# danilodjor/fault-tolerant-llm-training

Measured on AMD Instinct MI355X. Metric: tokens/sec/GPU seq-len 2048 DP at 1/2/4/8 MI355X; checkpoint save wall-clock (s), higher is better.
Workload: dtype bf16; 1 GPU; model=llama3-8b, global_batch=1, seq_len=2048, parallelism=dp1

## Files before the change

csrc/kernels/embedding.hip:

```cpp
#include "torch_utils.h"

#include <algorithm>

namespace {

__global__ __launch_bounds__(256) void emb_fwd_kernel(const int64_t* __restrict__ tok,
                                                      const char* __restrict__ w,
                                                      char* __restrict__ out, int T, int row_bytes) {
  const int row = blockIdx.x;
  const int64_t t = tok[row];
  const uint4* src = reinterpret_cast<const uint4*>(w + t * (long)row_bytes);
  uint4* dst = reinterpret_cast<uint4*>(out + (long)row * row_bytes);
  for (int c = threadIdx.x; c < row_bytes / 16; c += blockDim.x) dst[c] = src[c];
}

constexpr int SORT_NT = 1024, SORT_W = SORT_NT / 64, SORT_BITS = 6, SORT_BINS = 1 << SORT_BITS;

__global__ __launch_bounds__(SORT_NT) void tok_sort_kernel(const int64_t* __restrict__ tok, int T, int passes,
                                                           int* __restrict__ keys, int* __restrict__ vals) {
  __shared__ int hist[SORT_BINS];
  __shared__ int start[SORT_BINS];
  __shared__ int rbase[SORT_BINS];
  __shared__ int wcnt[SORT_W][SORT_BINS];
  const int tid = threadIdx.x, lane = tid & 63, wid = tid >> 6;
// ... 26 lines not shown
      const int d = (k >> shift) & (SORT_BINS - 1);
      unsigned long long m = __ballot(valid);
#pragma unroll
      for (int b = 0; b < SORT_BITS; ++b) {
        const unsigned long long bb = __ballot(valid && ((d >> b) & 1));
        m &= ((d >> b) & 1) ? bb : ~bb;
      }
      const int rank = __popcll(m & lower);
      wcnt[wid][lane] = 0;
      __syncthreads();
      if (valid && rank == 0) wcnt[wid][d] = __popcll(m);
      __syncthreads();
      if (tid < SORT_BINS) {
        int s = 0;
        for (int w = 0; w < SORT_W; ++w) {
          const int c = wcnt[w][tid];
          wcnt[w][tid] = s;
          s += c;
        }
        rbase[tid] = start[tid];
        start[tid] += s;
      }
      __syncthreads();
      if (valid) {
        const int pos = rbase[d] + wcnt[wid][d] + rank;
        dk[pos] = k;
        dv[pos] = v;
      }
      __syncthreads();
    }
  }
}

template <class E>
__global__ __launch_bounds__(256) void emb_bwd_kernel(const int* __restrict__ sorted_tok,
                                                      const int* __restrict__ perm,
                                                      const typename E::T* __restrict__ dy,
                                                      typename E::T* __restrict__ dw, int T, int D,
                                                      bool accumulate) {
  const int wave = (blockIdx.x * blockDim.x + threadIdx.x) >> 6;
  const int lane = threadIdx.x & 63;
  if (wave >= T) return;
  const int t = sorted_tok[wave];
  if (wave > 0 && sorted_tok[wave - 1] == t) return;
  int end = wave + 1;
  while (end < T && sorted_tok[end] == t) ++end;
  typename E::T* dst = dw + t * (long)D;
  for (int c = lane * 8; c < D; c += 64 * 8) {
    float acc[8] = {0, 0, 0, 0, 0, 0, 0, 0};
    for (int k = wave; k < end; ++k) {
      float x[8];
      ld8<E>(dy + perm[k] * (long)D + c, x);
#pragma unroll
      for (int j = 0; j < 8; ++j) acc[j] += x[j];
    }
    if (accumulate) {
      float o[8];
      ld8<E>(dst + c, o);
#pragma unroll
      for (int j = 0; j < 8; ++j) acc[j] += o[j];
    }
    st8<E>(dst + c, acc);
  }
}

template <class E>
__global__ __launch_bounds__(256) void emb_bwd_sq_kernel(const int* __restrict__ sorted_tok,
                                                         const int* __restrict__ perm,
                                                         const typename E::T* __restrict__ dy,
                                                         typename E::T* __restrict__ dw, int T, int D,
                                                         float* __restrict__ part, int nparts) {
  __shared__ float red[4];
  const int lane = threadIdx.x & 63, wid = threadIdx.x >> 6;
  float sq = 0.f;
  for (int wave = blockIdx.x * 4 + wid; wave < T; wave += gridDim.x * 4) {
    const int t = sorted_tok[wave];
    if (wave > 0 && sorted_tok[wave - 1] == t) continue;
    int end = wave + 1;
    while (end < T && sorted_tok[end] == t) ++end;
    typename E::T* dst = dw + t * (long)D;
    for (int c = lane * 8; c < D; c += 64 * 8) {
      float acc[8] = {0, 0, 0, 0, 0, 0, 0, 0};
      for (int k = wave; k < end; ++k) {
        float x[8];
        ld8<E>(dy + perm[k] * (long)D + c, x);
#pragma unroll
        for (int j = 0; j < 8; ++j) acc[j] += x[j];
      }
      const P8<E> r = pk8<E>(acc);
      *reinterpret_cast<uint4*>(dst + c) = r.v[0];
      if constexpr (!E::is16) *reinterpret_cast<uint4*>(dst + c + 4) = r.v[1];
      float st[8];
      unp8<E>(r, st);
#pragma unroll
      for (int j = 0; j < 8; ++j) sq = fmaf(st[j], st[j], sq);
    }
  }
  const float tot = block_sum<256>(sq, red);
  if (threadIdx.x == 0) part[blockIdx.x] = tot;
  for (long i = blockIdx.x + (long)gridDim.x * (1 + threadIdx.x); i < nparts; i += (long)gridDim.x * 256)
    part[i] = 0.f;
}

}

at::Tensor embedding_fwd(const at::Tensor& tokens, const at::Tensor& weight) {
  FT_CHECK_CUDA(weight);
  FT_CHECK_MODEL_DTYPE(weight);
  FT_CHECK_CONTIG(weight);
  FT_CHECK_CONTIG(tokens);
  TORCH_CHECK(tokens.scalar_type() == at::kLong, "embedding: tokens must be int64");
  const int D = weight.size(1);
  TORCH_CHECK(D % 8 == 0, "embedding: dim must be a multiple of 8");
  const int T = tokens.numel();
  const at::DeviceGuard guard(weight.device());
  auto sizes = tokens.sizes().vec();
  sizes.push_back(D);
  auto out = at::empty(sizes, weight.options());
  if (T > 0)
    hipLaunchKernelGGL(emb_fwd_kernel, dim3(T), dim3(256), 0, ft_stream(), cptr<int64_t>(tokens),
                       cptr<char>(weight), mptr<char>(out), T, (int)(D * weight.element_size()));
  FT_LAUNCH_CHECK();
  return out;
}

void embedding_bwd_(const at::Tensor& dy, const at::Tensor& tokens, const at::Tensor& dw,
                    bool accumulate, const std::optional<at::Tensor>& part) {
  FT_CHECK_CUDA(dy);
  FT_CHECK_MODEL_DTYPE(dy);
  TORCH_CHECK(dy.scalar_type() == dw.scalar_type(), "embedding_bwd: dtype mismatch");
  FT_CHECK_CONTIG(dy);
  FT_CHECK_CONTIG(dw);
  const int D = dw.size(1);
  const int T = tokens.numel();
  TORCH_CHECK(dy.numel() == (long)T * D, "embedding_bwd: shape mismatch");
  const at::DeviceGuard guard(dw.device());
  TORCH_CHECK(tokens.scalar_type() == at::kLong, "embedding_bwd: tokens must be int64");
  const long V = dw.size(0);
  TORCH_CHECK(V >= 1 && V < (1L << 30), "embedding_bwd: vocabulary size out of range");
  int bits = 1;
  while ((1L << bits) < V) ++bits;
  const int passes = (bits + SORT_BITS - 1) / SORT_BITS;
  auto flat = tokens.reshape({-1}).contiguous();
  if (!accumulate) FT_HIP_CHECK(hipMemsetAsync(dw.data_ptr(), 0, dw.nbytes(), ft_stream()));
  if (T > 0) {
    auto kv = at::empty({4, (long)T}, tokens.options().dtype(at::kInt));
    int* keys = mptr<int>(kv);
    int* vals = keys + 2L * T;
    hipLaunchKernelGGL(tok_sort_kernel, dim3(1), dim3(SORT_NT), 0, ft_stream(), cptr<int64_t>(flat), T, passes,
                       keys, vals);
    FT_LAUNCH_CHECK();
    const long fin = (long)((passes - 1) & 1) * T;
    const int blocks = (T * 64 + 255) / 256;
    const bool sq = part.has_value() && part->defined();
    if (sq) {
      TORCH_CHECK(!accumulate, "embedding_bwd: norm partials need a fresh gradient");
      FT_CHECK_F32((*part));
      FT_CHECK_CONTIG((*part));
      const int np = (int)part->numel();
      const int g = std::max(1, std::min({blocks, 256, np}));
      FT_DISPATCH_E(dy.scalar_type(),
                    hipLaunchKernelGGL(emb_bwd_sq_kernel<E>, dim3(g), dim3(256), 0, ft_stream(), keys + fin,
                                       vals + fin, cptr<typename E::T>(dy), mptr<typename E::T>(dw), T, D,
                                       mptr<float>(*part), np));
    } else {
      FT_DISPATCH_E(dy.scalar_type(),
                    hipLaunchKernelGGL(emb_bwd_kernel<E>, dim3(blocks), dim3(256), 0, ft_stream(), keys + fin,
                                       vals + fin, cptr<typename E::T>(dy), mptr<typename E::T>(dw), T, D,
                                       accumulate));
    }
  } else if (part.has_value() && part->defined()) {
    part->zero_();
  }
  FT_LAUNCH_CHECK();
}

TORCH_LIBRARY_FRAGMENT(ftamd, m) {
  m.def("embedding_fwd(Tensor tokens, Tensor weight) -> Tensor", &embedding_fwd);
  m.def("embedding_bwd_(Tensor dy, Tensor tokens, Tensor(a!) dw, bool accumulate, Tensor(b!)? part=None) -> ()",
        &embedding_bwd_);
}
```

csrc/kernels/optim.hip:

```cpp
#include "torch_utils.h"

#include <vector>

#include <cstdlib>

namespace {

typedef unsigned int u32x4_t __attribute__((ext_vector_type(4)));

template <bool NT>
__device__ __forceinline__ uint4 ld16(const void* p) {
  if constexpr (NT) {
    const u32x4_t v = __builtin_nontemporal_load(reinterpret_cast<const u32x4_t*>(p));
    return make_uint4(v.x, v.y, v.z, v.w);
  } else {
    return *reinterpret_cast<const uint4*>(p);
  }
}

template <bool NT>
__device__ __forceinline__ void st16(void* p, uint4 v) {
  if constexpr (NT) {
    const u32x4_t w = {v.x, v.y, v.z, v.w};
    __builtin_nontemporal_store(w, reinterpret_cast<u32x4_t*>(p));
// ... 33 lines not shown
  }
  __shared__ float red[4];
  s = block_sum<256>(s, red);
  if (threadIdx.x == 0) partial[blockIdx.x] = s;
}

__global__ __launch_bounds__(1024) void norm_finish_kernel(const float* __restrict__ partial,
                                                           int np, float extra_sumsq_scale,
                                                           float max_norm,
                                                           float* __restrict__ stats) {
  float s = 0.f;
  const int n4 = np >> 2;
  const float4* p4 = reinterpret_cast<const float4*>(partial);
  if ((reinterpret_cast<uintptr_t>(partial) & 15) == 0) {
    for (int i = threadIdx.x; i < n4; i += 1024) {
      const float4 v = p4[i];
      s += (v.x + v.y) + (v.z + v.w);
    }
    for (int i = 4 * n4 + threadIdx.x; i < np; i += 1024) s += partial[i];
  } else {
    for (int i = threadIdx.x; i < np; i += 1024) s += partial[i];
  }
  __shared__ float red[16];
  s = block_sum<1024>(s, red);
  if (threadIdx.x == 0) {
    const float norm = sqrtf(s * extra_sumsq_scale);
    stats[0] = norm;
    const bool bad = !isfinite(norm);
    stats[1] = (max_norm > 0.f && !bad) ? fminf(1.f, max_norm / (norm + 1e-6f)) : 1.f;
    stats[2] = (bad || stats[2] != 0.f) ? 1.f : 0.f;
  }
}

template <class P, class S, bool NT>
__global__ __launch_bounds__(256) void adamw_kernel(typename P::T* __restrict__ p,
                                                    const typename P::T* __restrict__ g,
                                                    typename S::T* __restrict__ m,
                                                    typename S::T* __restrict__ v,
                                                    long n8, float lr, float beta1, float beta2,
                                                    float eps, float wd, float inv_bc1,
                                                    float inv_sqrt_bc2,
                                                    const float* __restrict__ stats,
                                                    const float* __restrict__ hyper, int exact) {
  if (stats[2] != 0.f) return;
  if (hyper != nullptr) {
    lr = hyper[0];
    inv_bc1 = hyper[1];
    inv_sqrt_bc2 = hyper[2];
  }
  const float coef = stats[1];
  const float decay = 1.f - lr * wd;
  const float step = lr * inv_bc1;
  for (long i = blockIdx.x * 256L + threadIdx.x; i < n8; i += (long)gridDim.x * 256) {
    float pf[8], gf[8], mf[8], vf[8];
    V8<P, NT>::load(p + i * 8, pf);
    V8<P, NT>::load(g + i * 8, gf);
    V8<S, NT>::load(m + i * 8, mf);
    V8<S, NT>::load(v + i * 8, vf);
#pragma unroll
    for (int j = 0; j < 8; ++j) {
      const float gj = gf[j] * coef;
      pf[j] *= decay;
      mf[j] += (gj - mf[j]) * (1.f - beta1);
      vf[j] = vf[j] * beta2 + (1.f - beta2) * gj * gj;
      if (exact) {
        const float denom = sqrtf(vf[j]) * inv_sqrt_bc2 + eps;
        pf[j] -= step * mf[j] / denom;
      } else {
        const float denom = fast_sqrt(vf[j]) * inv_sqrt_bc2 + eps;
        pf[j] -= step * mf[j] * fast_rcp(denom);
      }
    }
    V8<P, NT>::store(p + i * 8, pf);
    V8<S, NT>::store(m + i * 8, mf);
    V8<S, NT>::store(v + i * 8, vf);
  }
}

int stream_grid(long n8) {
  long g = (n8 + 255) / 256;
  return (int)std::max(1L, std::min(g, 65535L));
}

void launch_sumsq(const at::Tensor& grad, long n8, int nb, float* partial) {
  const bool nt = stream_nt();
  FT_DISPATCH_E(grad.scalar_type(), {
    if (nt)
      hipLaunchKernelGGL((sumsq_kernel<E, true>), dim3(nb), dim3(256), 0, ft_stream(),
                         cptr<typename E::T>(grad), n8, partial);
    else
      hipLaunchKernelGGL((sumsq_kernel<E, false>), dim3(nb), dim3(256), 0, ft_stream(),
                         cptr<typename E::T>(grad), n8, partial);
  });
}

}

void grad_norm_(const at::Tensor& grad, const at::Tensor& stats, double max_norm) {
  FT_CHECK_CUDA(grad);
  FT_CHECK_CONTIG(grad);
  FT_CHECK_F32(stats);
  TORCH_CHECK(grad.numel() % 8 == 0, "grad_norm: numel must be a multiple of 8");
  const at::DeviceGuard guard(grad.device());
  const long n8 = grad.numel() / 8;
  const int nb = std::max(1, std::min(NORM_BLOCKS, (int)((n8 + 255) / 256)));
  auto partial = at::empty({nb}, grad.options().dtype(at::kFloat));
  launch_sumsq(grad, n8, nb, mptr<float>(partial));
  FT_LAUNCH_CHECK();
  hipLaunchKernelGGL(norm_finish_kernel, dim3(1), dim3(1024), 0, ft_stream(), cptr<float>(partial), nb,
                     1.f, (float)max_norm, mptr<float>(stats));
  FT_LAUNCH_CHECK();
}

void adamw_(const at::Tensor& p, const at::Tensor& g, const at::Tensor& m, const at::Tensor& v,
            const at::Tensor& stats, double lr, double beta1, double beta2, double eps, double wd,
            int64_t step, int64_t max_blocks, const std::optional<at::Tensor>& hyper) {
  const float* hp = nullptr;
  if (hyper.has_value() && hyper->defined()) {
    FT_CHECK_F32((*hyper));
    TORCH_CHECK(hyper->is_cuda() && hyper->numel() >= 3, "adamw: hyper must be a device fp32[3]");
    hp = cptr<float>(*hyper);
  }
  FT_CHECK_CUDA(p);
  FT_CHECK_CONTIG(p);
  FT_CHECK_CONTIG(g);
  FT_CHECK_CONTIG(m);
  FT_CHECK_CONTIG(v);
  FT_CHECK_F32(stats);
  TORCH_CHECK(p.numel() == g.numel() && p.numel() == m.numel() && p.numel() == v.numel(),
              "adamw: size mismatch");
  TORCH_CHECK(p.numel() % 8 == 0, "adamw: numel must be a multiple of 8");
  TORCH_CHECK(p.scalar_type() == g.scalar_type() && m.scalar_type() == v.scalar_type(),
              "adamw: dtype mismatch");
  const at::DeviceGuard guard(p.device());
  const long n8 = p.numel() / 8;
  const float bc1 = 1.f - (float)std::pow(beta1, (double)step);
  const float bc2 = 1.f - (float)std::pow(beta2, (double)step);
  const float inv_bc1 = 1.f / bc1, inv_sqrt_bc2 = 1.f / std::sqrt(bc2);
  int nb = stream_grid(n8);
  if (max_blocks > 0) nb = (int)std::max(1L, std::min((n8 + 255) / 256, (long)max_blocks));
  const dim3 grid(nb), block(256);
  const bool nt = stream_nt();
  TORCH_CHECK(m.scalar_type() == p.scalar_type() || m.scalar_type() == at::kFloat,
              "adamw: optimizer states must have the parameter dtype or fp32");
  const int exact = (int)ft_exact_math() || p.scalar_type() == at::kFloat;
  auto go = [&](auto ptag, auto stag) {
    using P = decltype(ptag);
    using S = decltype(stag);
    using PT = typename P::T;
    using ST = typename S::T;
    if (nt)
      hipLaunchKernelGGL((adamw_kernel<P, S, true>), grid, block, 0, ft_stream(), mptr<PT>(p),
                         cptr<PT>(g), mptr<ST>(m), mptr<ST>(v), n8, (float)lr, (float)beta1,
                         (float)beta2, (float)eps, (float)wd, inv_bc1, inv_sqrt_bc2,
                         cptr<float>(stats), hp, exact);
    else
      hipLaunchKernelGGL((adamw_kernel<P, S, false>), grid, block, 0, ft_stream(), mptr<PT>(p),
                         cptr<PT>(g), mptr<ST>(m), mptr<ST>(v), n8, (float)lr, (float)beta1,
                         (float)beta2, (float)eps, (float)wd, inv_bc1, inv_sqrt_bc2,
                         cptr<float>(stats), hp, exact);
  };
  FT_DISPATCH_E(p.scalar_type(), {
    if (m.scalar_type() == at::kFloat) go(E{}, EF32{});
    else go(E{}, E{});
  });
  FT_LAUNCH_CHECK();
}

void sumsq_into_(const at::Tensor& grad, const at::Tensor& partial) {
  FT_CHECK_CUDA(grad);
  FT_CHECK_CONTIG(grad);
  FT_CHECK_F32(partial);
  FT_CHECK_CONTIG(partial);
  TORCH_CHECK(grad.numel() % 8 == 0, "sumsq_into: numel must be a multiple of 8");
  TORCH_CHECK(partial.numel() >= 1 && partial.numel() <= 65535, "sumsq_into: bad partial size");
  const at::DeviceGuard guard(grad.device());
  const long n8 = grad.numel() / 8;
  const int nb = (int)partial.numel();
  launch_sumsq(grad, n8, nb, mptr<float>(partial));
  FT_LAUNCH_CHECK();
}

void norm_finish_(const at::Tensor& partial, const at::Tensor& stats, double max_norm) {
  FT_CHECK_CUDA(partial);
  FT_CHECK_F32(partial);
  FT_CHECK_F32(stats);
  const at::DeviceGuard guard(partial.device());
  hipLaunchKernelGGL(norm_finish_kernel, dim3(1), dim3(1024), 0, ft_stream(), cptr<float>(partial),
                     (int)partial.numel(), 1.f, (float)max_norm, mptr<float>(stats));
  FT_LAUNCH_CHECK();
}

int64_t cu_masked_stream(int64_t stride, int64_t phase) {
  TORCH_CHECK(stride >= 1 && phase >= 0 && phase < stride, "cu_masked_stream: 0 <= phase < stride");
  int dev = 0, ncu = 0;
  FT_HIP_CHECK(hipGetDevice(&dev));
  FT_HIP_CHECK(hipDeviceGetAttribute(&ncu, hipDeviceAttributeMultiprocessorCount, dev));
  std::vector<uint32_t> mask((ncu + 31) / 32, 0u);
  for (int c = (int)phase; c < ncu; c += (int)stride) mask[c / 32] |= 1u << (c % 32);
  hipStream_t st = nullptr;
  FT_HIP_CHECK(hipExtStreamCreateWithCUMask(&st, (uint32_t)mask.size(), mask.data()));
  return reinterpret_cast<int64_t>(st);
}

TORCH_LIBRARY_FRAGMENT(ftamd, m) {
  m.def("cu_masked_stream(int stride, int phase=0) -> int", &cu_masked_stream);
  m.def("sumsq_into_(Tensor grad, Tensor(a!) partial) -> ()", &sumsq_into_);
  m.def("norm_finish_(Tensor partial, Tensor(a!) stats, float max_norm) -> ()", &norm_finish_);
  m.def("grad_norm_(Tensor grad, Tensor(a!) stats, float max_norm) -> ()", &grad_norm_);
  m.def(
      "adamw_(Tensor(a!) p, Tensor g, Tensor(b!) m, Tensor(c!) v, Tensor stats, float lr, float "
      "beta1, float beta2, float eps, float wd, int step, int max_blocks=0, Tensor? hyper=None) -> ()",
      &adamw_);
}
```

fault_tolerant_llm_training_amd/ckpt/state.py:

```python
from __future__ import annotations

import hashlib
from collections import OrderedDict
from dataclasses import asdict
from typing import Any, Dict, Optional

import torch

from .format import FORMAT_TAG, strip_compile_prefix


def layout_hash(model) -> str:
    flat = model.flat
    h = hashlib.sha1()
    for name, s in flat.slots.items():
        h.update(f"{name}:{s.shape}:{s.offset};".encode())
    h.update(str(flat.dtype).encode())
    return h.hexdigest()[:16]


def _view(buf: torch.Tensor, s) -> torch.Tensor:
    return buf[s.offset : s.offset + s.numel].view(s.shape)


# ... 25 lines not shown
    }
    if rng is not None:
        out["rng"] = rng
    return out


def _flat_source(tensors, slots, numel: int, dtype) -> Optional[torch.Tensor]:
    base = None
    for name, t in tensors.items():
        s = slots.get(name)
        if s is None or t.dtype != dtype or tuple(t.shape) != tuple(s.shape) or not t.is_contiguous():
            return None
        st = t.untyped_storage()
        if base is None:
            base = st
        elif st.data_ptr() != base.data_ptr():
            return None
        if t.storage_offset() != s.offset:
            return None
    if base is None or base.nbytes() < numel * torch.tensor([], dtype=dtype).element_size():
        return None
    return torch.empty(0, dtype=dtype).set_(base)[:numel]


@torch.no_grad()
def restore_model(model, sd: Dict[str, torch.Tensor]) -> str:
    flat = model.flat
    sd = strip_compile_prefix(sd)
    expected = list(model.state_dict().keys())
    missing = [k for k in expected if k not in sd]
    unexpected = [k for k in sd if k not in flat.slots]
    if missing or unexpected:
        raise KeyError(f"checkpoint/model mismatch: missing={missing[:5]} unexpected={unexpected[:5]}")
    src = _flat_source(sd, flat.slots, flat.numel, flat.dtype)
    if src is not None:
        from .restore import h2d

        h2d(flat.params, src)
        return "flat"
    for name in expected:
        _view(flat.params, flat.slots[name]).copy_(sd[name], non_blocking=True)
    return "per-tensor"


def capture_rng(device: torch.device) -> Dict[str, Any]:
    r = {"torch": torch.get_rng_state()}
    if device.type == "cuda":
        r["cuda"] = torch.cuda.get_rng_state(device)
    return r


def restore_rng(r: Optional[Dict[str, Any]], device: torch.device) -> None:
    if not r:
        return
    if "torch" in r:
        torch.set_rng_state(r["torch"])
    if device.type == "cuda" and "cuda" in r:
        torch.cuda.set_rng_state(r["cuda"], device)


def shard_regions(model, optimizer, rank: int, world: int, align: int = 2048):
    from .engine import Region

    flat = model.flat
    P = flat.numel

# ... 15 lines not shown
```

fault_tolerant_llm_training_amd/ops/functional.py:

```python
from __future__ import annotations

import collections
import functools
import os
from typing import Optional

import torch
import torch.nn.functional as F

from .._native import kernels, native
from .grad_sink import GradSink

IGNORE_INDEX = -100

_BLAS_ONLY = os.environ.get("FT_GEMM_BLAS", "0") == "1"
_W4_FWD = True
_W4_BWD = os.environ.get("FT_W4_BWD", "1") != "0"
_W4_DTYPES = (torch.bfloat16, torch.float16)
_F32_MFMA = os.environ.get("FT_F32_MFMA", "1") != "0"


def set_f32_mfma(on: bool) -> None:
    global _F32_MFMA
    _F32_MFMA = bool(on)
# ... 210 lines not shown

def join_dw_stream() -> None:
    if _dw_streams:
        cur = torch.cuda.current_stream()
        k = _dev_key(cur.device)
        s = _dw_streams.get(k)
        if s is not None:
            cur.wait_stream(s)
            q = _dw_pending.get(k)
            if q:
                q.clear()


def norm_bwd_into_sink(dy, x, w, rstd, mean, sink: GradSink, dres=None) -> torch.Tensor:
    dx = kernels().norm_bwd(dy, x, w, rstd, mean, sink.buf, dres, sink.accumulate, sink.part)
    if sink.part is not None:
        sink.sq_done = True
    sink.ready()
    return dx


def _write_weight_grad(sink: Optional[GradSink], g: torch.Tensor):
    if sink is None:
        return g
    sink.set_(g.to(sink.buf.dtype))
    return None


class EmbeddingFn(torch.autograd.Function):
    @staticmethod
    def forward(ctx, tokens, weight, sink):
        ctx.sink = sink
        ctx.vocab = weight.shape[0]
        ctx.save_for_backward(tokens)
        ctx.wshape = weight.shape
        if native(weight):
            return kernels().embedding_fwd(tokens.contiguous(), weight)
        return F.embedding(tokens, weight)

    @staticmethod
    def backward(ctx, dy):
        (tokens,) = ctx.saved_tensors
        sink = ctx.sink
        dy = dy.contiguous()
        if sink is not None and sink.gather is not None:
            if sink.defer:
                sink.stash.append((tokens.reshape(-1), dy.reshape(-1, dy.shape[-1])))
                return None, None, None
            if sink.stash:
                tokens = torch.cat([t for t, _ in sink.stash] + [tokens.reshape(-1)])
                dy = torch.cat([g for _, g in sink.stash] + [dy.reshape(-1, dy.shape[-1])])
                sink.stash = []
            tokens, dy = sink.gather(tokens, dy)
        if native(dy):
            if sink is None:
                dw = torch.zeros(ctx.wshape, dtype=dy.dtype, device=dy.device)
                kernels().embedding_bwd_(dy, tokens.contiguous(), dw, False)
                return None, dw, None
            part = sink.part if (sink.part is not None and not sink.accumulate) else None
            kernels().embedding_bwd_(dy, tokens.contiguous(), sink.buf, sink.accumulate, part)
            if part is not None:
                sink.sq_done = True
            sink.ready()
            return None, None, None
        dw = torch.zeros(ctx.wshape, dtype=torch.float32, device=dy.device)
        if dy.is_cuda:
            dw.index_put_((tokens.reshape(-1),), dy.reshape(-1, ctx.wshape[1]).float(), accumulate=True)
        else:
            dw.index_add_(0, tokens.reshape(-1), dy.reshape(-1, ctx.wshape[1]).float())
        return None, _write_weight_grad(sink, dw.to(dy.dtype)), None


def embedding(tokens, weight, sink=None):
    return EmbeddingFn.apply(tokens, weight, sink)


def norm_reference(x: torch.Tensor, w: torch.Tensor, eps: float, layernorm: bool) -> torch.Tensor:
    xf = x.float()
    if layernorm:
        xf = xf - xf.mean(-1, keepdim=True)
    n = xf * torch.rsqrt(xf.pow(2).mean(-1, keepdim=True) + eps)
    return n.type_as(x) * w


class NormFn(torch.autograd.Function):
    @staticmethod
    def forward(ctx, x, weight, sink, eps, layernorm):
        ctx.sink, ctx.eps, ctx.ln = sink, eps, layernorm
        if native(x):
            xc = x.contiguous()
            y, rstd, mean = kernels().norm_fwd(xc, weight, eps, layernorm)
            ctx.save_for_backward(xc, weight, rstd, mean)
            return y
# ... 360 lines not shown
```

fault_tolerant_llm_training_amd/ops/grad_sink.py:

```python
from __future__ import annotations

from typing import Callable, Optional

import torch


class GradSink:
    __slots__ = ("buf", "start", "end", "accumulate", "hook", "name", "gather", "defer", "stash", "part", "sq_done")

    def __init__(self, buf: torch.Tensor, start: int = 0, end: int = 0, name: str = ""):
        self.buf = buf
        self.start = start
        self.end = end
        self.accumulate = False
        self.hook: Optional[Callable[["GradSink"], None]] = None
        self.name = name
        self.gather: Optional[Callable] = None
        self.defer = False
        self.stash: list = []
        self.part: Optional[torch.Tensor] = None
        self.sq_done = False

    def ready(self) -> None:
        if self.hook is not None:
            self.hook(self)

    def mm(self, a: torch.Tensor, b: torch.Tensor) -> None:
        out = self.buf.view(a.shape[0], b.shape[1])
        if self.accumulate:
            out.addmm_(a, b)
        else:
            torch.mm(a, b, out=out)
        self.ready()

    def set_(self, g: torch.Tensor) -> None:
        if self.accumulate:
            self.buf.add_(g.view_as(self.buf))
        else:
            self.buf.copy_(g.view_as(self.buf))
        self.ready()


def sink_of(p: torch.Tensor) -> Optional[GradSink]:
    return getattr(p, "_ft_sink", None)
```

fault_tolerant_llm_training_amd/optim/adamw.py:

```python
from __future__ import annotations

import math
from typing import List, Optional, Tuple

import torch
import torch.distributed as dist

from .._native import kernels, native
from ..models.flat import FlatParamSpace


class NonFiniteGradError(RuntimeError):
    pass


class ParamGate:

    def __init__(self):
        self.entries: List[list] = []

    def add(self, lo: int, hi: int, handle) -> None:
        self.entries.append([lo, hi, handle])

    def wait(self, lo: int, hi: int) -> None:
# ... 55 lines not shown
        name_of = {id(p): n for n, p in flat.param_objs.items()}
        self._index_slots = [flat.slots[name_of[id(p)]] for p in params]

    def clip_grad_norm_(self, max_norm: Optional[float] = None) -> torch.Tensor:
        if max_norm is not None:
            self.max_grad_norm = float(max_norm)
        return self.stats[0]

    def _stream_ctx(self):
        r = self.reducer
        if r is not None and r.overlap:
            return torch.cuda.stream(r.side)
        import contextlib

        return contextlib.nullcontext()

    def _hyper(self):
        grp = self.param_groups[0]
        b1, b2 = grp["betas"]
        return float(grp["lr"]), b1, b2, grp["eps"], grp["weight_decay"]

    def stage_hyper(self, step: int) -> None:
        import numpy as np

        lr, b1, b2, _eps, _wd = self._hyper()
        bc1 = np.float32(1.0) - np.float32(b1 ** step)
        bc2 = np.float32(1.0) - np.float32(b2 ** step)
        h = self._hyper_ring[self._hyper_i % len(self._hyper_ring)]
        self._hyper_i += 1
        h.copy_(torch.from_numpy(np.array([np.float32(lr), np.float32(1.0) / bc1,
                                           np.float32(1.0) / np.sqrt(bc2)], dtype=np.float32)))
        self.hyper.copy_(h, non_blocking=True)

    def _update(self, p, g, m, v, lr, b1, b2, eps, wd, max_blocks: int = 0):
        if native(p):
            kernels().adamw_(p, g, m, v, self.stats, lr, b1, b2, eps, wd, self.step_count, max_blocks,
                             self.hyper if self.graph_mode else None)
        else:
            _adamw_reference(p, g, m, v, self.stats, lr, b1, b2, eps, wd, self.step_count)

    @torch.no_grad()
    def step(self, closure=None):
        self.step_count += 1
        lr, b1, b2, eps, wd = self._hyper()
        f = self.flat
        r = self.reducer
        cuda = f.params.is_cuda
        if r is None:
            if cuda:
                from ..ops.functional import join_dw_stream

                join_dw_stream()
            if native(f.grads):
                kernels().grad_norm_(f.grads, self.stats, self.max_grad_norm)
            else:
                gd = f.grads.double() if f.grads.dtype == torch.float64 else f.grads.float()
                _norm_reference(gd.pow(2).sum().reshape(1), self.stats, self.max_grad_norm)
            self._update(f.params, f.grads, self.exp_avg, self.exp_avg_sq, lr, b1, b2, eps, wd)
            self._publish_stats()
            return None
        if r.overlap:
            r.side.wait_stream(torch.cuda.current_stream())
        with self._stream_ctx():
            total = r.global_sumsq()
            if cuda:
                kernels().norm_finish_(total, self.stats, self.max_grad_norm)
            else:
                _norm_reference(total.sum().reshape(1), self.stats, self.max_grad_norm)
            if not self.graph_mode:
                self._publish_stats()
            for b in sorted(r.buckets, key=lambda b: b.lo):
                slo, shi = r.state_range(b)
                self._update(r.param_for_update(b), r.grad_for_update(b), self.exp_avg[slo:shi],
                             self.exp_avg_sq[slo:shi], lr, b1, b2, eps, wd,
                             self.overlap_blocks if r.overlap else 0)
                if self.zero1 and r.dry_comm:
                    pass
                elif self.zero1 and r.single_stream and r.overlap:
                    dist.all_gather_into_tensor(f.params[b.lo : b.hi], r.param_shard(b), group=r.group)
                    b.agevent.record()
                    self.gate.add(b.lo, b.hi, b.agevent)
                elif self.zero1:
                    work = dist.all_gather_into_tensor(f.params[b.lo : b.hi], r.param_shard(b),
                                                       group=r.group, async_op=True)
                    if r.overlap:
                        self.gate.add(b.lo, b.hi, work)
                    else:
                        work.wait()
                elif r.overlap:
                    b.event.record()
                    self.gate.add(b.lo, b.hi, b.event)
        return None

    def _publish_stats(self):
        i = self.step_count % self.RING
        h = self._ring[i]
        if self.stats.is_cuda:
            h.copy_(self.stats, non_blocking=True)
            ev = self._ring_events[i]
            if ev is None:
                ev = self._ring_events[i] = torch.cuda.Event()
            ev.record()
            self._stats_event = ev
        else:
            h.copy_(self.stats)
        self._ring_steps[i] = self.step_count
        self._stats_step = self.step_count

# ... 165 lines not shown
```

fault_tolerant_llm_training_amd/parallel/ddp.py:

```python
from __future__ import annotations

import os
from typing import List, Optional

import torch
import torch.distributed as dist

from .._native import kernels, native
from ..models.flat import FlatParamSpace
from ..ops.grad_sink import GradSink

MODES = ("local", "allreduce", "zero1")
LOCAL_BUCKET_MB = 64.0
DP_BUCKET_MB = 256.0
PARTIALS_PER_BUCKET = 512
SUMSQ_AT_END = False


def set_sumsq_at_end(on: bool) -> None:
    global SUMSQ_AT_END
    SUMSQ_AT_END = bool(on)


FUSED_SUMSQ = True


def set_fused_sumsq(on: bool) -> None:
    global FUSED_SUMSQ
    FUSED_SUMSQ = bool(on)


def sink_partials(numel: int, ndim: int, shape=None, tile_rows: int = 256) -> int:
    if ndim <= 1:
        return max(1, (numel + 31) // 32)
    n = max(1, (numel + 32767) // 32768)
    if shape is not None and len(shape) == 2:
        n = max(n, -(-int(shape[0]) // tile_rows) * -(-int(shape[1]) // 128))
    return n


def _copy_back(dst: torch.Tensor, src: torch.Tensor, temps) -> None:
    dst.copy_(src)
    if src.is_cuda:
        cur = torch.cuda.current_stream(src.device)
        for t in temps:
            t.record_stream(cur)


# ... 109 lines not shown
        for sink in self._sq_sinks:
            lo, hi = sink.part
            sink.part = self.partials[lo:hi]
            sink.sq_done = False
            self._sq_slices.append(sink.part)
        self._sq_slice_of = {id(s): t for s, t in zip(self._sq_sinks, self._sq_slices)}
        self.sumsq_total = torch.zeros(1, dtype=torch.float32, device=flat.device)
        self.shard_numel = 0
        if mode == "zero1":
            for b in sorted(self.buckets, key=lambda b: b.lo):
                b.shard_len = b.numel // self.world
                b.shard_lo = self.shard_numel
                self.shard_numel += b.shard_len
        self.side = torch.cuda.Stream(device=flat.device) if self.overlap else None
        self.comm = self.world > 1 or mode != "local"
        self.single_stream = False
        if not self.fused_sumsq:
            for sink in list(flat.sinks.values()) + list(extra_sinks):
                sink.part, sink.sq_done = None, False
        if self.cuda:
            for b in self.buckets:
                b.event = torch.cuda.Event()
                b.agevent = torch.cuda.Event()
        self._extra_sinks = list(extra_sinks)
        for sink in list(flat.sinks.values()) + list(extra_sinks):
            sink.hook = self._on_ready
        self._pending_sumsq: List[Bucket] = []
        self._next = 0
        self.fault_after_buckets = 0
        self.dry_comm = False
        self.sync = True
        self.gathered = False
        self.emb_sink = flat.sinks.get(emb) if self.sparse_embedding else None

    def param_shard(self, b: Bucket) -> torch.Tensor:
        lo = b.lo + self.rank * b.shard_len
        return self.flat.params[lo : lo + b.shard_len]

    def grad_shard(self, b: Bucket) -> torch.Tensor:
        lo = b.lo + self.rank * b.shard_len
        return self.flat.grads[lo : lo + b.shard_len]

    def grad_for_update(self, b: Bucket) -> torch.Tensor:
        if self.mode == "zero1":
            return self.grad_shard(b)
        return self.flat.grads[b.lo : b.hi]

    def _gather_rows(self, tokens: torch.Tensor, dy: torch.Tensor):
        self.gathered = True
        t = tokens.reshape(-1).contiguous()
        d = dy.reshape(t.numel(), -1).contiguous()
        if self.dry_comm:
            return t, d
        t_all = torch.empty(self.world * t.numel(), dtype=t.dtype, device=t.device)
        d_all = torch.empty(self.world * d.shape[0], d.shape[1], dtype=d.dtype, device=d.device)
        if self.single_stream and self.overlap:
            cur = torch.cuda.current_stream()
            self.side.wait_stream(cur)
            with torch.cuda.stream(self.side):
                dist.all_gather_into_tensor(t_all, t, group=self.group)
                dist.all_gather_into_tensor(d_all, d, group=self.group)
            cur.wait_stream(self.side)
            for x in (t, d, t_all, d_all):
                x.record_stream(self.side)
            return t_all, d_all
        dist.all_gather_into_tensor(t_all, t, group=self.group)
# ... 75 lines not shown
        if native(g):
            kernels().sumsq_into_(g, part)
        else:
            part.zero_()
            part[0] = (g.double() if g.dtype == torch.float64 else g.float()).pow(2).sum()

    def _launch(self, b: Bucket) -> None:
        if self.cuda:
            from ..ops.functional import active_dw_stream

            dws = active_dw_stream(self.flat.device)
            if dws is not None and dws != torch.cuda.current_stream():
                dws.wait_stream(torch.cuda.current_stream())
                with torch.cuda.stream(dws):
                    self._launch_now(b)
                return
        self._launch_now(b)

    def _collective_blocking(self, b: Bucket, grads: torch.Tensor) -> None:
        if self.reduce_fp32:
            src = grads.float()
            if self.mode == "allreduce":
                dist.all_reduce(src, op=dist.ReduceOp.SUM, group=self.group)
                grads.copy_(src)
            else:
                out = src.new_empty(b.shard_len)
                dist.reduce_scatter_tensor(out, src, op=dist.ReduceOp.SUM, group=self.group)
                self.grad_shard(b).copy_(out)
        elif self.mode == "allreduce":
            dist.all_reduce(grads, op=dist.ReduceOp.SUM, group=self.group)
        elif self.mode == "zero1":
            dist.reduce_scatter_tensor(self.grad_shard(b), grads, op=dist.ReduceOp.SUM, group=self.group)

    def _launch_now(self, b: Bucket) -> None:
        b.launched = True
        grads = self.flat.grads[b.lo : b.hi]
        if self.single_stream and self.overlap:
            side = self.side
            b.event.record()
            side.wait_event(b.event)
            with torch.cuda.stream(side):
                if not (b.sparse or self.dry_comm):
                    self._collective_blocking(b, grads)
                if SUMSQ_AT_END:
                    self._pending_sumsq.append(b)
                else:
                    self._sumsq(self.grad_for_update(b), b)
            return
        if b.sparse or self.dry_comm:
            pass
        elif self.reduce_fp32:
            src = grads.float()
            if self.mode == "allreduce":
                b.work = dist.all_reduce(src, op=dist.ReduceOp.SUM, group=self.group, async_op=True)
                b.post = lambda: _copy_back(grads, src, (src,))
            else:
                out = src.new_empty(b.shard_len)
                b.work = dist.reduce_scatter_tensor(out, src, op=dist.ReduceOp.SUM, group=self.group,
                                                    async_op=True)
                shard = self.grad_shard(b)
                b.post = lambda: _copy_back(shard, out, (src, out))
        elif self.mode == "allreduce":
            b.work = dist.all_reduce(grads, op=dist.ReduceOp.SUM, group=self.group, async_op=True)
        elif self.mode == "zero1":
            b.work = dist.reduce_scatter_tensor(self.grad_shard(b), grads, op=dist.ReduceOp.SUM,
                                                group=self.group, async_op=True)
        if not self.overlap:
            return
        side = self.side
        if b.work is None:
            b.event.record()
            side.wait_event(b.event)
        with torch.cuda.stream(side):
            if b.work is not None:
                b.work.wait()
                b.work = None
                self._post(b)
            if SUMSQ_AT_END:
                self._pending_sumsq.append(b)
            else:
                self._sumsq(self.grad_for_update(b), b)
# ... 6 lines not shown

    def finish(self) -> None:
        if self.cuda:
            from ..ops.functional import join_dw_stream

            join_dw_stream()
        while self._next < len(self.buckets):
            b = self.buckets[self._next]
            self._next += 1
            self._launch(b)
        if self._pending_sumsq:
            with torch.cuda.stream(self.side):
                for b in self._pending_sumsq:
                    self._sumsq(self.grad_for_update(b), b)
            self._pending_sumsq = []
        if not self.overlap:
            for b in self.buckets:
                if b.work is not None:
                    b.work.wait()
                    b.work = None
                    self._post(b)
                self._sumsq(self.grad_for_update(b), b)
        for b in self.buckets:
            b.filled = 0
            b.launched = False
        self._next = 0
        self.gathered = False

    @torch.no_grad()
    def poison_and_complete(self, tokens_shape=None, dim: int = 0) -> None:
        self.sync = True
        nan = float("nan")
        poisoned = False
        for b in self.buckets[self._next:]:
            self.flat.grads[b.lo : b.hi].fill_(nan)
            poisoned = True
        while self._next < len(self.buckets) and not self.buckets[self._next].sparse:
            b = self.buckets[self._next]
            self._next += 1
            self._launch(b)
        if self.sparse_embedding and not self.gathered:
            T = 1
            for s_ in tokens_shape or (1,):
                T *= int(s_)
            tok = torch.zeros(T, dtype=torch.long, device=self.flat.device)
            dy = torch.full((T, dim), nan, dtype=self.flat.dtype, device=self.flat.device)
            self._gather_rows(tok, dy)
            es = self.emb_sink
            self.flat.grads[es.start : es.end].fill_(nan)
            poisoned = True
        del poisoned
        self.finish()

    def global_sumsq(self) -> torch.Tensor:
        if self.mode != "zero1":
            return self.partials
        if self.cuda:
            torch.sum(self.partials, dim=0, keepdim=True, out=self.sumsq_total)
        else:
            self.sumsq_total.copy_(self.partials.sum().reshape(1))
        if not self.dry_comm:
            dist.all_reduce(self.sumsq_total, op=dist.ReduceOp.SUM, group=self.group)
        return self.sumsq_total

    @torch.no_grad()
    def broadcast_params(self, src: int = 0) -> None:
# ... 10 lines not shown
```

Baseline: 20780 tokens/s (whole job, sum over GPUs).

## Sparse-zero embedding grad rows and skip untouched rows in AdamW

The embedding backward records which vocabulary rows it wrote, keeping a row list and a bitmap. On the next step it zeroes only the stale rows, replacing a full memset of the vocab×dim gradient. AdamW uses the bitmap to skip loading gradient values for untouched embedding rows, and the token sort moves into the forward pass so backward can reuse it. This adds validity tracking, which collectives, checkpoint loads and poisoning invalidate, and it risks stale gradients if any other writer to the buffer is missed.

New measurement: 20810 tokens/s (whole job, sum over GPUs) (median of 6 runs). Within noise of the previous version (+0.1%).

```diff
diff --git a/csrc/kernels/embedding.hip b/csrc/kernels/embedding.hip
--- a/csrc/kernels/embedding.hip
+++ b/csrc/kernels/embedding.hip
@@ -82,17 +82,52 @@
   }
 }
 
+
+__global__ __launch_bounds__(256) void emb_zero_stale_kernel(const int* __restrict__ rec, int cap,
+                                                             int* __restrict__ bits,
+                                                             const int* __restrict__ sorted_tok, int T,
+                                                             char* __restrict__ dw, long V, int row_bytes) {
+  const int lane = threadIdx.x & 63;
+  const int n = min(max(rec[0], 0), cap);
+  for (int i = blockIdx.x * 4 + (threadIdx.x >> 6); i < n; i += gridDim.x * 4) {
+    const int r = rec[1 + i];
+    if (i > 0 && rec[i] == r) continue;
+    if (r < 0 || r >= V) continue;
+    if (lane == 0) atomicAnd(&bits[r >> 5], ~(1 << (r & 31)));
+    int lo = 0, hi = T;
+    while (lo < hi) {
+      const int mid = (lo + hi) >> 1;
+      if (sorted_tok[mid] < r) lo = mid + 1;
+      else hi = mid;
+    }
+    if (lo < T && sorted_tok[lo] == r) continue;
+    uint4* dst = reinterpret_cast<uint4*>(dw + r * (long)row_bytes);
+    for (int c = lane; c < row_bytes / 16; c += 64) dst[c] = make_uint4(0, 0, 0, 0);
+  }
+}
+
+__device__ __forceinline__ void emb_record(int* __restrict__ rec, int* __restrict__ bits, int wave, int t,
+                                           bool head, int T, int lane) {
+  if (rec == nullptr || lane != 0) return;
+  rec[1 + wave] = t;
+  if (wave == 0) rec[0] = T;
+  if (head) atomicOr(&bits[t >> 5], 1 << (t & 31));
+}
+
 template <class E>
 __global__ __launch_bounds__(256) void emb_bwd_kernel(const int* __restrict__ sorted_tok,
                                                       const int* __restrict__ perm,
                                                       const typename E::T* __restrict__ dy,
                                                       typename E::T* __restrict__ dw, int T, int D,
-                                                      bool accumulate) {
+                                                      bool accumulate, int* __restrict__ rec,
+                                                      int* __restrict__ bits) {
   const int wave = (blockIdx.x * blockDim.x + threadIdx.x) >> 6;
   const int lane = threadIdx.x & 63;
   if (wave >= T) return;
   const int t = sorted_tok[wave];
-  if (wave > 0 && sorted_tok[wave - 1] == t) return;
+  const bool head = wave == 0 || sorted_tok[wave - 1] != t;
+  emb_record(rec, bits, wave, t, head, T, lane);
+  if (!head) return;
   int end = wave + 1;
   while (end < T && sorted_tok[end] == t) ++end;
   typename E::T* dst = dw + t * (long)D;
@@ -119,13 +154,16 @@
                                                          const int* __restrict__ perm,
                                                          const typename E::T* __restrict__ dy,
                                                          typename E::T* __restrict__ dw, int T, int D,
-                                                         float* __restrict__ part, int nparts) {
+                                                         float* __restrict__ part, int nparts,
+                                                         int* __restrict__ rec, int* __restrict__ bits) {
   __shared__ float red[4];
   const int lane = threadIdx.x & 63, wid = threadIdx.x >> 6;
   float sq = 0.f;
   for (int wave = blockIdx.x * 4 + wid; wave < T; wave += gridDim.x * 4) {
     const int t = sorted_tok[wave];
-    if (wave > 0 && sorted_tok[wave - 1] == t) continue;
+    const bool head = wave == 0 || sorted_tok[wave - 1] != t;
+    emb_record(rec, bits, wave, t, head, T, lane);
+    if (!head) continue;
     int end = wave + 1;
     while (end < T && sorted_tok[end] == t) ++end;
     typename E::T* dst = dw + t * (long)D;
@@ -174,8 +212,38 @@
   return out;
 }
 
-void embedding_bwd_(const at::Tensor& dy, const at::Tensor& tokens, const at::Tensor& dw,
-                    bool accumulate, const std::optional<at::Tensor>& part) {
+namespace {
+
+int sort_passes(long V) {
+  TORCH_CHECK(V >= 1 && V < (1L << 30), "embedding: vocabulary size out of range");
+  int bits = 1;
+  while ((1L << bits) < V) ++bits;
+  return (bits + SORT_BITS - 1) / SORT_BITS;
+}
+
+}
+
+at::Tensor token_sort(const at::Tensor& tokens, int64_t V) {
+  FT_CHECK_CUDA(tokens);
+  TORCH_CHECK(tokens.scalar_type() == at::kLong, "token_sort: tokens must be int64");
+  const int passes = sort_passes(V);
+  const at::DeviceGuard guard(tokens.device());
+  auto flat = tokens.reshape({-1}).contiguous();
+  const int T = flat.numel();
+  auto kv = at::empty({4, (long)T}, tokens.options().dtype(at::kInt));
+  if (T > 0) {
+    int* keys = mptr<int>(kv);
+    hipLaunchKernelGGL(tok_sort_kernel, dim3(1), dim3(SORT_NT), 0, ft_stream(), cptr<int64_t>(flat), T, passes,
+                       keys, keys + 2L * T);
+    FT_LAUNCH_CHECK();
+  }
+  return kv;
+}
+
+bool embedding_bwd_(const at::Tensor& dy, const at::Tensor& tokens, const at::Tensor& dw,
+                    bool accumulate, const std::optional<at::Tensor>& part,
+                    const std::optional<at::Tensor>& sorted, const std::optional<at::Tensor>& rows,
+                    const std::optional<at::Tensor>& row_bits, bool rows_valid) {
   FT_CHECK_CUDA(dy);
   FT_CHECK_MODEL_DTYPE(dy);
   TORCH_CHECK(dy.scalar_type() == dw.scalar_type(), "embedding_bwd: dtype mismatch");
@@ -183,24 +251,55 @@
   FT_CHECK_CONTIG(dw);
   const int D = dw.size(1);
   const int T = tokens.numel();
+  TORCH_CHECK(D % 8 == 0, "embedding_bwd: dim must be a multiple of 8");
   TORCH_CHECK(dy.numel() == (long)T * D, "embedding_bwd: shape mismatch");
   const at::DeviceGuard guard(dw.device());
   TORCH_CHECK(tokens.scalar_type() == at::kLong, "embedding_bwd: tokens must be int64");
   const long V = dw.size(0);
-  TORCH_CHECK(V >= 1 && V < (1L << 30), "embedding_bwd: vocabulary size out of range");
-  int bits = 1;
-  while ((1L << bits) < V) ++bits;
-  const int passes = (bits + SORT_BITS - 1) / SORT_BITS;
-  auto flat = tokens.reshape({-1}).contiguous();
-  if (!accumulate) FT_HIP_CHECK(hipMemsetAsync(dw.data_ptr(), 0, dw.nbytes(), ft_stream()));
+  const int passes = sort_passes(V);
+  int* rec = nullptr;
+  int* bits = nullptr;
+  int cap = 0;
+  if (!accumulate && rows.has_value() && rows->defined()) {
+    TORCH_CHECK(row_bits.has_value() && row_bits->defined(), "embedding_bwd: rows without row_bits");
+    TORCH_CHECK(rows->is_cuda() && rows->scalar_type() == at::kInt && rows->is_contiguous() && rows->numel() >= 1,
+                "embedding_bwd: rows must be a device int32 [1 + capacity]");
+    TORCH_CHECK(row_bits->is_cuda() && row_bits->scalar_type() == at::kInt && row_bits->is_contiguous() &&
+                    row_bits->numel() * 32 >= V,
+                "embedding_bwd: row_bits must be a device int32 with a bit per row");
+    cap = (int)std::min<long>(rows->numel() - 1, 1L << 30);
+    if (T <= cap) {
+      rec = mptr<int>(*rows);
+      bits = mptr<int>(*row_bits);
+    }
+  }
+  const bool sparse_zero = rec != nullptr && rows_valid;
+  if (!accumulate && !sparse_zero) {
+    FT_HIP_CHECK(hipMemsetAsync(dw.data_ptr(), 0, dw.nbytes(), ft_stream()));
+    if (rec != nullptr) FT_HIP_CHECK(hipMemsetAsync(bits, 0, row_bits->nbytes(), ft_stream()));
+  }
+  at::Tensor kv;
+  const int* keys = nullptr;
+  const int* vals = nullptr;
   if (T > 0) {
-    auto kv = at::empty({4, (long)T}, tokens.options().dtype(at::kInt));
-    int* keys = mptr<int>(kv);
-    int* vals = keys + 2L * T;
-    hipLaunchKernelGGL(tok_sort_kernel, dim3(1), dim3(SORT_NT), 0, ft_stream(), cptr<int64_t>(flat), T, passes,
-                       keys, vals);
+    if (sorted.has_value() && sorted->defined()) {
+      kv = *sorted;
+      TORCH_CHECK(kv.is_cuda() && kv.scalar_type() == at::kInt && kv.is_contiguous() && kv.numel() == 4L * T,
+                  "embedding_bwd: sorted must be token_sort's int32 [4, T]");
+    } else {
+      kv = token_sort(tokens, V);
+    }
+    const long fin = (long)((passes - 1) & 1) * T;
+    keys = cptr<int>(kv) + fin;
+    vals = cptr<int>(kv) + 2L * T + fin;
+  }
+  if (sparse_zero) {
+    const int g = std::max(1, std::min(256, (cap + 3) / 4));
+    hipLaunchKernelGGL(emb_zero_stale_kernel, dim3(g), dim3(256), 0, ft_stream(), rec, cap, bits, keys, T,
+                       mptr<char>(dw), V, (int)(D * dw.element_size()));
     FT_LAUNCH_CHECK();
-    const long fin = (long)((passes - 1) & 1) * T;
+  }
+  if (T > 0) {
     const int blocks = (T * 64 + 255) / 256;
     const bool sq = part.has_value() && part->defined();
     if (sq) {
@@ -210,23 +309,28 @@
       const int np = (int)part->numel();
       const int g = std::max(1, std::min({blocks, 256, np}));
       FT_DISPATCH_E(dy.scalar_type(),
-                    hipLaunchKernelGGL(emb_bwd_sq_kernel<E>, dim3(g), dim3(256), 0, ft_stream(), keys + fin,
-                                       vals + fin, cptr<typename E::T>(dy), mptr<typename E::T>(dw), T, D,
-                                       mptr<float>(*part), np));
+                    hipLaunchKernelGGL(emb_bwd_sq_kernel<E>, dim3(g), dim3(256), 0, ft_stream(), keys, vals,
+                                       cptr<typename E::T>(dy), mptr<typename E::T>(dw), T, D,
+                                       mptr<float>(*part), np, rec, bits));
     } else {
       FT_DISPATCH_E(dy.scalar_type(),
-                    hipLaunchKernelGGL(emb_bwd_kernel<E>, dim3(blocks), dim3(256), 0, ft_stream(), keys + fin,
-                                       vals + fin, cptr<typename E::T>(dy), mptr<typename E::T>(dw), T, D,
-                                       accumulate));
-    }
-  } else if (part.has_value() && part->defined()) {
-    part->zero_();
+                    hipLaunchKernelGGL(emb_bwd_kernel<E>, dim3(blocks), dim3(256), 0, ft_stream(), keys, vals,
+                                       cptr<typename E::T>(dy), mptr<typename E::T>(dw), T, D, accumulate,
+                                       rec, bits));
+    }
+  } else {
+    if (part.has_value() && part->defined()) part->zero_();
+    if (rec != nullptr) FT_HIP_CHECK(hipMemsetAsync(rec, 0, sizeof(int), ft_stream()));
   }
   FT_LAUNCH_CHECK();
+  return rec != nullptr;
 }
 
 TORCH_LIBRARY_FRAGMENT(ftamd, m) {
   m.def("embedding_fwd(Tensor tokens, Tensor weight) -> Tensor", &embedding_fwd);
-  m.def("embedding_bwd_(Tensor dy, Tensor tokens, Tensor(a!) dw, bool accumulate, Tensor(b!)? part=None) -> ()",
-        &embedding_bwd_);
-}
+  m.def("token_sort(Tensor tokens, int vocab) -> Tensor", &token_sort);
+  m.def(
+      "embedding_bwd_(Tensor dy, Tensor tokens, Tensor(a!) dw, bool accumulate, Tensor(b!)? part=None, "
+      "Tensor? sorted=None, Tensor(c!)? rows=None, Tensor(d!)? row_bits=None, bool rows_valid=False) -> bool",
+      &embedding_bwd_);
+}
diff --git a/csrc/kernels/optim.hip b/csrc/kernels/optim.hip
--- a/csrc/kernels/optim.hip
+++ b/csrc/kernels/optim.hip
@@ -89,7 +89,7 @@
   }
 }
 
-template <class P, class S, bool NT>
+template <class P, class S, bool NT, bool MASK>
 __global__ __launch_bounds__(256) void adamw_kernel(typename P::T* __restrict__ p,
                                                     const typename P::T* __restrict__ g,
                                                     typename S::T* __restrict__ m,
@@ -98,7 +98,9 @@
                                                     float eps, float wd, float inv_bc1,
                                                     float inv_sqrt_bc2,
                                                     const float* __restrict__ stats,
-                                                    const float* __restrict__ hyper, int exact) {
+                                                    const float* __restrict__ hyper, int exact,
+                                                    const int* __restrict__ bits, long lo8, long hi8,
+                                                    unsigned row8) {
   if (stats[2] != 0.f) return;
   if (hyper != nullptr) {
     lr = hyper[0];
@@ -111,7 +113,19 @@
   for (long i = blockIdx.x * 256L + threadIdx.x; i < n8; i += (long)gridDim.x * 256) {
     float pf[8], gf[8], mf[8], vf[8];
     V8<P, NT>::load(p + i * 8, pf);
-    V8<P, NT>::load(g + i * 8, gf);
+    bool has = true;
+    if constexpr (MASK) {
+      if (i >= lo8 && i < hi8) {
+        const unsigned row = (unsigned)(i - lo8) / row8;
+        has = (bits[row >> 5] >> (row & 31)) & 1;
+      }
+    }
+    if (has) {
+      V8<P, NT>::load(g + i * 8, gf);
+    } else {
+#pragma unroll
+      for (int j = 0; j < 8; ++j) gf[j] = 0.f;
+    }
     V8<S, NT>::load(m + i * 8, mf);
     V8<S, NT>::load(v + i * 8, vf);
 #pragma unroll
@@ -171,7 +185,8 @@
 
 void adamw_(const at::Tensor& p, const at::Tensor& g, const at::Tensor& m, const at::Tensor& v,
             const at::Tensor& stats, double lr, double beta1, double beta2, double eps, double wd,
-            int64_t step, int64_t max_blocks, const std::optional<at::Tensor>& hyper) {
+            int64_t step, int64_t max_blocks, const std::optional<at::Tensor>& hyper,
+            const std::optional<at::Tensor>& row_bits, int64_t row_len, int64_t mask_lo, int64_t mask_hi) {
   const float* hp = nullptr;
   if (hyper.has_value() && hyper->defined()) {
     FT_CHECK_F32((*hyper));
@@ -201,21 +216,40 @@
   TORCH_CHECK(m.scalar_type() == p.scalar_type() || m.scalar_type() == at::kFloat,
               "adamw: optimizer states must have the parameter dtype or fp32");
   const int exact = (int)ft_exact_math() || p.scalar_type() == at::kFloat;
+  const int* bits = nullptr;
+  long lo8 = 0, hi8 = 0;
+  unsigned row8 = 1;
+  if (row_bits.has_value() && row_bits->defined() && mask_hi > 0 && mask_lo < p.numel()) {
+    TORCH_CHECK(row_bits->is_cuda() && row_bits->scalar_type() == at::kInt && row_bits->is_contiguous(),
+                "adamw: row_bits must be a device int32 bitmap");
+    TORCH_CHECK(row_len >= 8 && row_len % 8 == 0 && mask_lo % 8 == 0 && mask_hi > mask_lo &&
+                    (mask_hi - mask_lo) % row_len == 0,
+                "adamw: the masked region must be whole rows of a multiple of 8 elements");
+    TORCH_CHECK(row_bits->numel() * 32 >= (mask_hi - mask_lo) / row_len, "adamw: row_bits too short");
+    if ((mask_hi - mask_lo) / 8 < (1L << 32) && row_len / 8 < (1L << 32)) {
+      bits = cptr<int>(*row_bits);
+      lo8 = mask_lo / 8;
+      hi8 = std::min<long>(mask_hi / 8, n8);
+      row8 = (unsigned)(row_len / 8);
+    }
+  }
   auto go = [&](auto ptag, auto stag) {
     using P = decltype(ptag);
     using S = decltype(stag);
     using PT = typename P::T;
     using ST = typename S::T;
-    if (nt)
-      hipLaunchKernelGGL((adamw_kernel<P, S, true>), grid, block, 0, ft_stream(), mptr<PT>(p),
-                         cptr<PT>(g), mptr<ST>(m), mptr<ST>(v), n8, (float)lr, (float)beta1,
-                         (float)beta2, (float)eps, (float)wd, inv_bc1, inv_sqrt_bc2,
-                         cptr<float>(stats), hp, exact);
-    else
-      hipLaunchKernelGGL((adamw_kernel<P, S, false>), grid, block, 0, ft_stream(), mptr<PT>(p),
-                         cptr<PT>(g), mptr<ST>(m), mptr<ST>(v), n8, (float)lr, (float)beta1,
-                         (float)beta2, (float)eps, (float)wd, inv_bc1, inv_sqrt_bc2,
-                         cptr<float>(stats), hp, exact);
+    auto launch = [&](auto kernel) {
+      hipLaunchKernelGGL(kernel, grid, block, 0, ft_stream(), mptr<PT>(p), cptr<PT>(g), mptr<ST>(m),
+                         mptr<ST>(v), n8, (float)lr, (float)beta1, (float)beta2, (float)eps, (float)wd,
+                         inv_bc1, inv_sqrt_bc2, cptr<float>(stats), hp, exact, bits, lo8, hi8, row8);
+    };
+    if (bits != nullptr) {
+      if (nt) launch(adamw_kernel<P, S, true, true>);
+      else launch(adamw_kernel<P, S, false, true>);
+    } else {
+      if (nt) launch(adamw_kernel<P, S, true, false>);
+      else launch(adamw_kernel<P, S, false, false>);
+    }
   };
   FT_DISPATCH_E(p.scalar_type(), {
     if (m.scalar_type() == at::kFloat) go(E{}, EF32{});
@@ -267,6 +301,7 @@
   m.def("grad_norm_(Tensor grad, Tensor(a!) stats, float max_norm) -> ()", &grad_norm_);
   m.def(
       "adamw_(Tensor(a!) p, Tensor g, Tensor(b!) m, Tensor(c!) v, Tensor stats, float lr, float "
-      "beta1, float beta2, float eps, float wd, int step, int max_blocks=0, Tensor? hyper=None) -> ()",
+      "beta1, float beta2, float eps, float wd, int step, int max_blocks=0, Tensor? hyper=None, "
+      "Tensor? row_bits=None, int row_len=0, int mask_lo=0, int mask_hi=0) -> ()",
       &adamw_);
 }
diff --git a/fault_tolerant_llm_training_amd/ckpt/state.py b/fault_tolerant_llm_training_amd/ckpt/state.py
--- a/fault_tolerant_llm_training_amd/ckpt/state.py
+++ b/fault_tolerant_llm_training_amd/ckpt/state.py
@@ -81,6 +81,8 @@
     unexpected = [k for k in sd if k not in flat.slots]
     if missing or unexpected:
         raise KeyError(f"checkpoint/model mismatch: missing={missing[:5]} unexpected={unexpected[:5]}")
+    for sink in flat.sinks.values():
+        sink.invalidate_rows()
     src = _flat_source(sd, flat.slots, flat.numel, flat.dtype)
     if src is not None:
         from .restore import h2d
diff --git a/fault_tolerant_llm_training_amd/ops/functional.py b/fault_tolerant_llm_training_amd/ops/functional.py
--- a/fault_tolerant_llm_training_amd/ops/functional.py
+++ b/fault_tolerant_llm_training_amd/ops/functional.py
@@ -266,15 +266,25 @@
     def forward(ctx, tokens, weight, sink):
         ctx.sink = sink
         ctx.vocab = weight.shape[0]
-        ctx.save_for_backward(tokens)
         ctx.wshape = weight.shape
         if native(weight):
-            return kernels().embedding_fwd(tokens.contiguous(), weight)
+            tok = tokens.contiguous()
+            out = kernels().embedding_fwd(tok, weight)
+            presort = ctx.needs_input_grad[1] and tok.numel() > 0 and (sink is None or sink.gather is None)
+            ctx.presorted = presort
+            if presort:
+                ctx.save_for_backward(tokens, kernels().token_sort(tok, weight.shape[0]))
+            else:
+                ctx.save_for_backward(tokens)
+            return out
+        ctx.presorted = False
+        ctx.save_for_backward(tokens)
         return F.embedding(tokens, weight)
 
     @staticmethod
     def backward(ctx, dy):
-        (tokens,) = ctx.saved_tensors
+        tokens = ctx.saved_tensors[0]
+        kv = ctx.saved_tensors[1] if ctx.presorted else None
         sink = ctx.sink
         dy = dy.contiguous()
         if sink is not None and sink.gather is not None:
@@ -289,10 +299,14 @@
         if native(dy):
             if sink is None:
                 dw = torch.zeros(ctx.wshape, dtype=dy.dtype, device=dy.device)
-                kernels().embedding_bwd_(dy, tokens.contiguous(), dw, False)
+                kernels().embedding_bwd_(dy, tokens.contiguous(), dw, False, None, kv)
                 return None, dw, None
             part = sink.part if (sink.part is not None and not sink.accumulate) else None
-            kernels().embedding_bwd_(dy, tokens.contiguous(), sink.buf, sink.accumulate, part)
+            valid = sink.rows_valid and not sink.accumulate
+            sink.rows_valid = False
+            wrote = kernels().embedding_bwd_(dy, tokens.contiguous(), sink.buf, sink.accumulate, part, kv,
+                                             sink.rows, sink.row_bits, valid)
+            sink.rows_valid = bool(wrote) and not sink.accumulate
             if part is not None:
                 sink.sq_done = True
             sink.ready()
diff --git a/fault_tolerant_llm_training_amd/ops/grad_sink.py b/fault_tolerant_llm_training_amd/ops/grad_sink.py
--- a/fault_tolerant_llm_training_amd/ops/grad_sink.py
+++ b/fault_tolerant_llm_training_amd/ops/grad_sink.py
@@ -6,7 +6,8 @@
 
 
 class GradSink:
-    __slots__ = ("buf", "start", "end", "accumulate", "hook", "name", "gather", "defer", "stash", "part", "sq_done")
+    __slots__ = ("buf", "start", "end", "accumulate", "hook", "name", "gather", "defer", "stash", "part", "sq_done",
+                 "rows", "row_bits", "rows_valid")
 
     def __init__(self, buf: torch.Tensor, start: int = 0, end: int = 0, name: str = ""):
         self.buf = buf
@@ -20,6 +21,9 @@
         self.stash: list = []
         self.part: Optional[torch.Tensor] = None
         self.sq_done = False
+        self.rows: Optional[torch.Tensor] = None
+        self.row_bits: Optional[torch.Tensor] = None
+        self.rows_valid = False
 
     def ready(self) -> None:
         if self.hook is not None:
@@ -27,13 +31,18 @@
 
     def mm(self, a: torch.Tensor, b: torch.Tensor) -> None:
         out = self.buf.view(a.shape[0], b.shape[1])
+        self.rows_valid = False
         if self.accumulate:
             out.addmm_(a, b)
         else:
             torch.mm(a, b, out=out)
         self.ready()
 
+    def invalidate_rows(self) -> None:
+        self.rows_valid = False
+
     def set_(self, g: torch.Tensor) -> None:
+        self.rows_valid = False
         if self.accumulate:
             self.buf.add_(g.view_as(self.buf))
         else:
diff --git a/fault_tolerant_llm_training_amd/optim/adamw.py b/fault_tolerant_llm_training_amd/optim/adamw.py
--- a/fault_tolerant_llm_training_amd/optim/adamw.py
+++ b/fault_tolerant_llm_training_amd/optim/adamw.py
@@ -111,12 +111,20 @@
                                            np.float32(1.0) / np.sqrt(bc2)], dtype=np.float32)))
         self.hyper.copy_(h, non_blocking=True)
 
-    def _update(self, p, g, m, v, lr, b1, b2, eps, wd, max_blocks: int = 0):
+    def _update(self, p, g, m, v, lr, b1, b2, eps, wd, max_blocks: int = 0, mask=None):
         if native(p):
+            bits, row_len, lo, hi = mask if mask is not None else (None, 0, 0, 0)
             kernels().adamw_(p, g, m, v, self.stats, lr, b1, b2, eps, wd, self.step_count, max_blocks,
-                             self.hyper if self.graph_mode else None)
+                             self.hyper if self.graph_mode else None, bits, row_len, lo, hi)
         else:
             _adamw_reference(p, g, m, v, self.stats, lr, b1, b2, eps, wd, self.step_count)
+
+    def _row_mask(self, lo: int, hi: int):
+        r = self.reducer
+        s = getattr(r, "row_sink", None) if r is not None else None
+        if s is None or not s.rows_valid or self.zero1 or hi <= s.start or lo >= s.end:
+            return None
+        return s.row_bits, int(s.buf.shape[1]), s.start - lo, s.end - lo
 
     @torch.no_grad()
     def step(self, closure=None):
@@ -152,7 +160,7 @@
                 slo, shi = r.state_range(b)
                 self._update(r.param_for_update(b), r.grad_for_update(b), self.exp_avg[slo:shi],
                              self.exp_avg_sq[slo:shi], lr, b1, b2, eps, wd,
-                             self.overlap_blocks if r.overlap else 0)
+                             self.overlap_blocks if r.overlap else 0, self._row_mask(b.lo, b.hi))
                 if self.zero1 and r.dry_comm:
                     pass
                 elif self.zero1 and r.single_stream and r.overlap:
diff --git a/fault_tolerant_llm_training_amd/parallel/ddp.py b/fault_tolerant_llm_training_amd/parallel/ddp.py
--- a/fault_tolerant_llm_training_amd/parallel/ddp.py
+++ b/fault_tolerant_llm_training_amd/parallel/ddp.py
@@ -14,6 +14,7 @@
 LOCAL_BUCKET_MB = 64.0
 DP_BUCKET_MB = 256.0
 PARTIALS_PER_BUCKET = 512
+EMB_ROWS_CAP = 8 * 2048
 SUMSQ_AT_END = False
 
 
@@ -189,6 +190,13 @@
         self.sync = True
         self.gathered = False
         self.emb_sink = flat.sinks.get(emb) if self.sparse_embedding else None
+        self.row_sink = flat.sinks.get(emb) if (self.cuda and native(flat.grads)) else None
+        if self.row_sink is not None:
+            s = self.row_sink
+            if s.rows is None:
+                s.rows = torch.zeros(1 + EMB_ROWS_CAP, dtype=torch.int32, device=flat.device)
+                s.row_bits = torch.zeros((s.buf.shape[0] + 31) // 32, dtype=torch.int32, device=flat.device)
+            s.rows_valid = False
 
     def param_shard(self, b: Bucket) -> torch.Tensor:
         lo = b.lo + self.rank * b.shard_len
@@ -330,6 +338,11 @@
         elif self.mode == "zero1":
             dist.reduce_scatter_tensor(self.grad_shard(b), grads, op=dist.ReduceOp.SUM, group=self.group)
 
+    def _foreign_write(self, b: Bucket) -> None:
+        s = self.row_sink
+        if s is not None and self.mode != "local" and b.lo < s.end and b.hi > s.start:
+            s.invalidate_rows()
+
     def _launch_now(self, b: Bucket) -> None:
         b.launched = True
         grads = self.flat.grads[b.lo : b.hi]
@@ -339,12 +352,15 @@
             side.wait_event(b.event)
             with torch.cuda.stream(side):
                 if not (b.sparse or self.dry_comm):
+                    self._foreign_write(b)
                     self._collective_blocking(b, grads)
                 if SUMSQ_AT_END:
                     self._pending_sumsq.append(b)
                 else:
                     self._sumsq(self.grad_for_update(b), b)
             return
+        if not (b.sparse or self.dry_comm):
+            self._foreign_write(b)
         if b.sparse or self.dry_comm:
             pass
         elif self.reduce_fp32:
@@ -417,6 +433,8 @@
         self.sync = True
         nan = float("nan")
         poisoned = False
+        if self.row_sink is not None:
+            self.row_sink.invalidate_rows()
         for b in self.buckets[self._next:]:
             self.flat.grads[b.lo : b.hi].fill_(nan)
             poisoned = True
```
